# run-llama/semtools

Hardware: AMD Instinct MI355X
Metric: chunk-vectors scanned/sec (whole job) (higher is better)
Workload: dtype f32; 1 GPU; c2: 1 query x 1M chunks (D=256, f32) per GPU, brute-force cosine + top-k; rows_per_gpu=1000000, dim=256, top_k=10, corpus_copies_rotated=2

## Files before the change

### include/semtools_hip.h

```cpp
#ifndef SEMTOOLS_HIP_H
#define SEMTOOLS_HIP_H

#include <stdint.h>

#ifdef __cplusplus
extern "C" {
#endif

#define SMT_OK 0
#define SMT_E_INVALID (-1)
#define SMT_E_HIP (-2)
#define SMT_E_NOMEM (-3)
#define SMT_E_TRUNCATED (-4)
#define SMT_E_IO (-5)
#define SMT_E_UNSUPPORTED (-6)

#define SMT_DIM 256u

#define SMT_MODE_DOCUMENTS 0
#define SMT_MODE_WORKSPACE 1

typedef struct smt_ctx smt_ctx;
typedef struct smt_model smt_model;
typedef struct smt_corpus smt_corpus;
// ... 350 lines not shown

int smt_debug_scan_pairs(smt_ctx *ctx, uint64_t *paired, uint64_t *alone, uint64_t *absorbed);

int smt_debug_scan_groups(smt_ctx *ctx, uint64_t *by_size );

int smt_debug_scan_groups_wide(smt_ctx *ctx, uint64_t *by_size );

int smt_debug_scan_groups_deep(smt_ctx *ctx, uint64_t *by_size );

int smt_debug_select_groups(smt_ctx *ctx, uint64_t *by_size );

int smt_debug_ov_ready(smt_ctx *ctx, uint64_t *records);

int smt_debug_host_timing(smt_ctx *ctx, uint64_t *ns , uint64_t *calls);

#define SMT_DEBUG_FAIL_STAGE 1
#define SMT_DEBUG_FAIL_AGREE 2
#define SMT_DEBUG_FAIL_BUILD 3
int smt_debug_group_fail_next(smt_group *group, int where, int code);

int smt_debug_batched_scores(smt_corpus *corpus, const float *queries, uint32_t nq, uint64_t first_row, uint32_t n_rows,
                             float *out);

int smt_debug_nominations(smt_corpus *corpus, const float *queries, uint32_t nq, uint32_t top_k, const smt_range *ranges, uint32_t n_ranges,
                          const float *tau, int buffered, float *out_dist, uint32_t *out_hits, uint32_t *out_counts, uint32_t *out_route);

int smt_debug_merge_sources(smt_ctx *ctx, const uint64_t *const *lists_dev, uint32_t n_lists, uint32_t nq, uint32_t k_in, uint32_t k_out,
                            uint64_t *out_packed_dev);
int smt_debug_merge_packed_strided(smt_ctx *ctx, const uint64_t *packed_dev, uint64_t list_stride_words, uint32_t n_lists, uint32_t nq,
                                   uint32_t k_in, uint32_t k_out, uint64_t *out_packed_dev);
// ... 25 lines not shown
```

### rust/src/search/hip_ffi.rs

```rust
#![allow(non_camel_case_types, dead_code)]
use std::os::raw::{c_char, c_int, c_void};

macro_rules! opaque { ($($name:ident),*) => { $( #[repr(C)] pub struct $name { _private: [u8; 0] } )* } }
opaque!(SmtCtx, SmtModel, SmtCorpus, SmtIvfpq, SmtGroup, SmtShardedCorpus, SmtShardedIvfpq, SmtShardedModel, SmtWordpiece, SmtUnigram, SmtLower);

#[repr(C)]
#[derive(Clone, Copy, Debug, PartialEq, Eq)]
pub struct SmtRange {
    pub begin: u64,
    pub end: u64,
}

#[repr(C)]
#[derive(Clone, Copy, Debug, Default)]
pub struct SmtIvfpqParams {
    pub nlist: u32,
    pub m: u32,
    pub nbits: u32,
    pub train_iters: u32,
    pub train_sample: u64,
    pub reserved: u32,
    pub local_pca: u32,
}

// ... 872 lines not shown
    pub fn smt_debug_range_sets(corpus: *const SmtCorpus, kept: *mut u64, hits: *mut u64, builds: *mut u64) -> c_int;
    pub fn smt_debug_image_tile(
        corpus: *mut SmtCorpus,
        tile: u64,
        out_tile_host: *mut c_void,
        out_zero_mask: *mut u32,
    ) -> c_int;
    pub fn smt_debug_deliveries(ctx: *mut SmtCtx, count: *mut u64) -> c_int;
    pub fn smt_debug_scan_pairs(ctx: *mut SmtCtx, paired: *mut u64, alone: *mut u64, absorbed: *mut u64) -> c_int;
    pub fn smt_debug_scan_groups(ctx: *mut SmtCtx, by_size: *mut u64) -> c_int;
    pub fn smt_debug_scan_groups_wide(ctx: *mut SmtCtx, by_size: *mut u64) -> c_int;
    pub fn smt_debug_scan_groups_deep(ctx: *mut SmtCtx, by_size: *mut u64) -> c_int;
    pub fn smt_debug_select_groups(ctx: *mut SmtCtx, by_size: *mut u64) -> c_int;
    pub fn smt_debug_ov_ready(ctx: *mut SmtCtx, records: *mut u64) -> c_int;
    pub fn smt_debug_host_timing(ctx: *mut SmtCtx, ns: *mut u64, calls: *mut u64) -> c_int;
    pub fn smt_debug_group_fail_next(group: *mut SmtGroup, where_: c_int, code: c_int) -> c_int;
    pub fn smt_debug_batched_scores(
        corpus: *mut SmtCorpus,
        queries: *const f32,
        nq: u32,
        first_row: u64,
        n_rows: u32,
        out: *mut f32,
    ) -> c_int;
    pub fn smt_debug_nominations(
        corpus: *mut SmtCorpus,
        queries: *const f32,
        nq: u32,
        top_k: u32,
        ranges: *const SmtRange,
// ... 86 lines not shown
```

### semtools_amd/_lib.py

```python
import ctypes as C
import os
import subprocess

import numpy as np

_HERE = os.path.dirname(os.path.abspath(__file__))
LIB_PATH = os.path.join(_HERE, "lib", "libsemtools_hip.so")

SMT_OK, SMT_E_INVALID, SMT_E_HIP, SMT_E_NOMEM, SMT_E_TRUNCATED, SMT_E_IO, SMT_E_UNSUPPORTED = 0, -1, -2, -3, -4, -5, -6
MODE_DOCUMENTS, MODE_WORKSPACE = 0, 1
DIM = 256

EXPORTS = [
    "smt_ctx_create", "smt_ctx_create_on_stream", "smt_ctx_aux_stream", "smt_ctx_destroy", "smt_ctx_synchronize", "smt_last_error", "smt_version",
    "smt_device_count", "smt_prof_enable", "smt_prof_reset", "smt_prof_read",
    "smt_model_create", "smt_model_create_from_file", "smt_model_create_from_device", "smt_model_destroy", "smt_embed", "smt_embed_device",
    "smt_corpus_create", "smt_corpus_from_device", "smt_corpus_destroy", "smt_corpus_append_host",
    "smt_corpus_write_rows", "smt_corpus_read_rows", "smt_corpus_truncate", "smt_corpus_rows", "smt_corpus_dim",
    "smt_corpus_prepack", "smt_corpus_image_bytes",
    "smt_corpus_save", "smt_corpus_load", "smt_corpus_append_to_file", "smt_search", "smt_search_topk_device", "smt_merge_topk",
    "smt_merge_topk_device", "smt_merge_topk_packed_device", "smt_ivfpq_build", "smt_ivfpq_destroy", "smt_ivfpq_search", "smt_ivfpq_search_device", "smt_ivfpq_search_ranges", "smt_ivfpq_search_ranges_device", "smt_ivfpq_search_wide", "smt_ivfpq_search_wide_device", "smt_ivfpq_info", "smt_ivfpq_list_sizes", "smt_ivfpq_save", "smt_ivfpq_load", "smt_ivfpq_append", "smt_ivfpq_compact", "smt_sharded_ivfpq_compact",
    "smt_set_tuning", "smt_fnv1a_hash", "smt_line_embedding_id", "smt_doc_meta_id",
    "smt_ctx_uncertain_count", "smt_debug_batched_scores",
    "smt_init", "smt_shutdown", "smt_default_group", "smt_group_create", "smt_group_create_logical", "smt_group_unique_id", "smt_group_create_rank",
# ... 2 lines not shown
    "smt_sharded_corpus_destroy", "smt_sharded_corpus_rows", "smt_sharded_corpus_rank_rows", "smt_sharded_corpus_shard",
    "smt_sharded_corpus_append_host", "smt_sharded_search", "smt_sharded_search_topk_device",
    "smt_sharded_ivfpq_build", "smt_sharded_ivfpq_destroy", "smt_sharded_ivfpq_shard", "smt_sharded_ivfpq_search", "smt_sharded_ivfpq_search_ranges", "smt_sharded_ivfpq_search_wide",
    "smt_group_from_ctx", "smt_sharded_corpus_create", "smt_sharded_corpus_load_layout", "smt_sharded_corpus_layout",
    "smt_sharded_corpus_append_to_file", "smt_sharded_corpus_read_rows", "smt_sharded_corpus_write_rows",
    "smt_sharded_model_create", "smt_sharded_model_create_from_file", "smt_sharded_model_destroy", "smt_sharded_embed",
    "smt_sharded_ivfpq_save", "smt_sharded_ivfpq_load", "smt_sharded_ivfpq_append", "smt_sharded_ivfpq_info",
    "smt_group_set_transport", "smt_group_transport", "smt_debug_range_sets", "smt_sharded_corpus_append_to_file_ex",
    "smt_debug_group_fail_next", "smt_search_topk_device_ex", "smt_sharded_search_topk_device_ex", "smt_debug_deliveries",
    "smt_corpus_compact", "smt_ctx_compact_stats", "smt_sharded_corpus_compact",
    "smt_model_create_typed", "smt_model_create_from_file_typed", "smt_model_create_from_device_typed", "smt_model_info",
    "smt_sharded_model_create_typed", "smt_sharded_model_create_from_file_typed", "smt_sharded_model_info",
    "smt_model_create_indexed", "smt_model_create_from_file_indexed", "smt_model_create_from_device_indexed", "smt_model_token_info",
    "smt_sharded_model_create_indexed", "smt_sharded_model_create_from_file_indexed", "smt_sharded_model_token_info",
    "smt_debug_scan_pairs", "smt_debug_image_tile", "smt_debug_scan_groups", "smt_debug_scan_groups_wide", "smt_debug_scan_groups_deep","smt_debug_nominations",
    "smt_debug_select_groups", "smt_debug_ov_ready", "smt_debug_host_timing",
    "smt_debug_merge_sources", "smt_debug_merge_packed_strided", "smt_debug_combine_status", "smt_debug_select_lists",
    "smt_debug_scan_lists", "smt_debug_scan_ring",
    "smt_wordpiece_create", "smt_wordpiece_create_utf8", "smt_wordpiece_info", "smt_wordpiece_destroy", "smt_wordpiece_scan_device", "smt_wordpiece_emit_device", "smt_wordpiece_tokenize",
    "smt_unigram_create", "smt_unigram_create_utf8", "smt_unigram_info", "smt_unigram_destroy", "smt_unigram_scan_device", "smt_unigram_emit_device", "smt_unigram_tokenize",
    "smt_unigram_set_long_pieces", "smt_unigram_long_stats", "smt_unigram_set_space_rules", "smt_unigram_set_long_rules",
    "smt_lower_tables_check", "smt_lower_create", "smt_lower_destroy", "smt_lower_device", "smt_lower_lines",
]
WP_NORMALIZER, WP_CLEAN_TEXT, WP_LOWERCASE = 1, 2, 4
WP_CP_ORDINARY, WP_CP_SPACE, WP_CP_ALONE, WP_CP_DROPPED, WP_CP_FLAG = 0, 1, 2, 3, 4
UG_MAX_WORD = 64
UG_MAX_LONG = 2048
UG_PREPEND = {"always": 0, "first": 1, "never": 2}
TABLE_F32, TABLE_F16, TABLE_I8 = 0, 1, 2
TABLE_DTYPES = {np.dtype(np.float32): TABLE_F32, np.dtype(np.float16): TABLE_F16, np.dtype(np.int8): TABLE_I8}
TABLE_NP = {v: k for k, v in TABLE_DTYPES.items()}
# ... 240 lines not shown
    L.smt_group_synchronize.argtypes = [vp]
    L.smt_group_barrier.argtypes = [vp]
    try:
        L.smt_debug_range_sets.argtypes = [vp, P(C.c_uint64), P(C.c_uint64), P(C.c_uint64)]
        L.smt_debug_group_fail_next.argtypes = [vp, i32, i32]
        L.smt_debug_deliveries.argtypes = [vp, P(C.c_uint64)]
        L.smt_debug_scan_pairs.argtypes = [vp, P(C.c_uint64), P(C.c_uint64), P(C.c_uint64)]
        L.smt_debug_image_tile.argtypes = [vp, u64, vp, P(C.c_uint32)]
        L.smt_debug_scan_groups.argtypes = [vp, P(C.c_uint64)]
        L.smt_debug_nominations.argtypes = [vp, vp, u32, u32, vp, u32, vp, i32, vp, vp, vp, P(C.c_uint32)]
        L.smt_debug_scan_groups_wide.argtypes = [vp, P(C.c_uint64)]
        L.smt_debug_scan_groups_deep.argtypes = [vp, P(C.c_uint64)]
        L.smt_debug_select_groups.argtypes = [vp, P(C.c_uint64)]
        L.smt_debug_ov_ready.argtypes = [vp, P(C.c_uint64)]
        L.smt_debug_host_timing.argtypes = [vp, P(C.c_uint64), P(C.c_uint64)]
        L.smt_debug_merge_sources.argtypes = [vp, P(vp), u32, u32, u32, u32, vp]
        L.smt_debug_merge_packed_strided.argtypes = [vp, vp, u64, u32, u32, u32, u32, vp]
        L.smt_debug_combine_status.argtypes = [vp, P(vp), vp, u64, u32, u32, vp]
        L.smt_debug_select_lists.argtypes = [vp, vp, u32, vp, u64, u32, u32, u32, i32, C.c_float, u64, f64, vp, u64, vp, vp, vp, vp, vp]
        L.smt_debug_scan_lists.argtypes = [vp, vp, u32, u32, vp, u32, vp, u64, P(C.c_uint32), P(C.c_uint32), P(C.c_uint32)]
        L.smt_debug_scan_ring.argtypes = [vp, u32, u64, vp]
    except AttributeError:
        pass
    L.smt_sharded_corpus_append_to_file_ex.argtypes = [vp, C.c_char_p, u64, u64, i32]
    L.smt_group_set_transport.argtypes = [vp, i32]
    L.smt_group_transport.argtypes = [vp]
    L.smt_sharded_corpus_from_host.argtypes = [vp, vp, u64, u32, P(vp)]
    L.smt_sharded_corpus_from_device.argtypes = [vp, P(vp), P(u64), u32, P(vp)]
    L.smt_sharded_corpus_load.argtypes = [vp, C.c_char_p, P(vp)]
    L.smt_sharded_corpus_save.argtypes = [vp, C.c_char_p]
# ... 108 lines not shown
```

### semtools_amd/core.py

```python
import collections
import ctypes as C
import math

import numpy as np

from . import _lib as L


CompactStats = collections.namedtuple("CompactStats", "calls rows_moved")


def _f32c(a):
    return np.ascontiguousarray(a, dtype=np.float32)


def _table(a):
    if not isinstance(a, np.ndarray):
        return _f32c(a)
    L.table_dtype_code(a.dtype)
    return np.ascontiguousarray(a)


def _open(obj):
    return getattr(obj, "_h", None) is not None and bool(obj._h)
# ... 64 lines not shown

    def select_groups(self):
        v = (C.c_uint64 * 17)()
        L.check(L.lib().smt_debug_select_groups(self._h, v))
        return tuple(int(x) for x in v)

    def ov_ready_records(self):
        n = C.c_uint64(0)
        L.check(L.lib().smt_debug_ov_ready(self._h, C.byref(n)))
        return int(n.value)

    def host_timing(self):
        v, n = (C.c_uint64 * 8)(), C.c_uint64(0)
        L.check(L.lib().smt_debug_host_timing(self._h, v, C.byref(n)))
        return tuple(int(x) for x in v), int(n.value)

    def compact_stats(self, reset=False):
        n, m = C.c_uint64(0), C.c_uint64(0)
        L.check(L.lib().smt_ctx_compact_stats(self._h, C.byref(n), C.byref(m), int(bool(reset))))
        return CompactStats(int(n.value), int(m.value))

    def aux_stream(self):
        st = C.c_void_p()
        L.check(L.lib().smt_ctx_aux_stream(self._h, C.byref(st)))
        return int(st.value or 0)

    def set_tuning(self, key, value):
        L.check(L.lib().smt_set_tuning(self._h, key.encode(), int(value)))

    def prof_enable(self, on=True):
# ... 992 lines not shown
```

### semtools_amd/csrc/api.cpp

```cpp
#include <algorithm>
#include <cerrno>
#include <cmath>
#include <limits>
#include <string>

#include <unistd.h>

#include "common.h"

namespace smt {

static thread_local char g_err[512] = "";

void set_error(const char *fmt, ...)
{
    va_list ap;
    va_start(ap, fmt);
    vsnprintf(g_err, sizeof(g_err), fmt, ap);
    va_end(ap);
}

int ensure_scratch(smt_ctx *ctx, size_t bytes)
{
    if (bytes <= ctx->scratch_bytes) return SMT_OK;
// ... 47 lines not shown
{
    if (!ctx->aux_stream || !ctx->ov_stream[0]) return SMT_OK;
    for (int b = 0; b < 2; ++b) {
        SMT_HIP_CHECK(hipEventRecord(ctx->ov_sel[b], ctx->ov_stream[b]));
        SMT_HIP_CHECK(hipStreamWaitEvent(ctx->aux_stream, ctx->ov_sel[b], 0));
    }
    return SMT_OK;
}

int drain_async(smt_ctx *ctx)
{
    if (!ctx->async_pending) return SMT_OK;
    ctx->async_pending = false;
    for (hipStream_t st : ctx->ov_stream)
        if (st) SMT_HIP_CHECK(hipStreamSynchronize(st));
    if (ctx->pair_live) {
        ctx->pair_live = false;
        unsigned long long gave_up = 0;
        SMT_HIP_CHECK(hipMemcpy(&gave_up, ctx->d_gate + 1, sizeof(gave_up), hipMemcpyDeviceToHost));
        if (gave_up) {
            (void)hipMemset(ctx->d_gate + 1, 0, sizeof(gave_up));
            set_error("scan_pair: a scan block gave up waiting for its launch's grouping decision");
            return SMT_E_HIP;
        }
    }
    if (!ctx->aux_stream || !ctx->d_flags) return SMT_OK;
    SMT_HIP_CHECK(hipStreamSynchronize(ctx->stream));
    SMT_HIP_CHECK(hipStreamSynchronize(ctx->aux_stream));
    unsigned long long timed_out = 0;
    SMT_HIP_CHECK(hipMemcpy(&timed_out, ctx->d_flags + 3, sizeof(timed_out), hipMemcpyDeviceToHost));
// ... 280 lines not shown
    if (ctx->aux_stream) { (void)hipStreamSynchronize(ctx->aux_stream); (void)hipStreamDestroy(ctx->aux_stream); }
    for (int b = 0; b < 2; ++b) {
        if (ctx->ov_stream[b]) { (void)hipStreamSynchronize(ctx->ov_stream[b]); (void)hipStreamDestroy(ctx->ov_stream[b]); }
        if (ctx->ov_ready[b]) (void)hipEventDestroy(ctx->ov_ready[b]);
        if (ctx->ov_sel[b]) (void)hipEventDestroy(ctx->ov_sel[b]);
    }
    if (ctx->ov_done) (void)hipEventDestroy(ctx->ov_done);
    if (ctx->d_gate) (void)hipFree(ctx->d_gate);
    if (ctx->d_pair_recs) (void)hipFree(ctx->d_pair_recs);
    if (ctx->d_wide_recs) (void)hipFree(ctx->d_wide_recs);
    if (ctx->d_deep_recs) (void)hipFree(ctx->d_deep_recs);
    if (ctx->h_pair_ring) (void)hipHostFree(ctx->h_pair_ring);
    if (ctx->d_deep_sel_recs) (void)hipFree(ctx->d_deep_sel_recs);
    if (ctx->d_sel_groups) (void)hipFree(ctx->d_sel_groups);
    if (ctx->h_sel_ring) (void)hipHostFree(ctx->h_sel_ring);
    if (ctx->d_flags) (void)hipFree(ctx->d_flags);
    if (ctx->d_status) (void)hipFree(ctx->d_status);
    if (ctx->d_steal) (void)hipFree(ctx->d_steal);
    for (auto &kv : ctx->prof)
        for (hipEvent_t ev : kv.second.ev) (void)hipEventDestroy(ev);
    if (ctx->d_scratch) (void)hipFree(ctx->d_scratch);
    if (ctx->d_largek) (void)hipFree(ctx->d_largek);
    if (ctx->d_embed_runs) (void)hipFree(ctx->d_embed_runs);
    if (ctx->h_pinned) (void)hipHostFree(ctx->h_pinned);
    if (ctx->h_pinned_in) (void)hipHostFree(ctx->h_pinned_in);
    if (ctx->h_ivf_ranges) (void)hipHostFree(ctx->h_ivf_ranges);
    if (ctx->ivf_ranges_up) (void)hipEventDestroy(ctx->ivf_ranges_up);
    if (ctx->d_stage) (void)hipFree(ctx->d_stage);
    if (ctx->own_stream) (void)hipStreamDestroy(ctx->stream);
    delete ctx;
// ... 22 lines not shown
    return SMT_OK;
} catch (...) { return smt::api_catch(); }

int smt_debug_scan_pairs(smt_ctx *ctx, uint64_t *paired, uint64_t *alone, uint64_t *absorbed)
try {
    int rc = check_ctx(ctx);
    if (rc) return rc;
    SMT_REQUIRE(paired && alone && absorbed, "null argument");
    if ((rc = bind_device(ctx))) return rc;
    SMT_HIP_CHECK(hipStreamSynchronize(ctx->stream));
    if ((rc = sync_side_streams(ctx))) return rc;
    unsigned long long v[3] = {0, 0, 0};
    if (ctx->d_gate) SMT_HIP_CHECK(hipMemcpy(v, ctx->d_gate + 2, sizeof(v), hipMemcpyDeviceToHost));
    *paired = v[0];
    *alone = v[1] + ctx->pair_alone_host;
    *absorbed = v[2];
    return SMT_OK;
} catch (...) { return smt::api_catch(); }

int smt_debug_scan_groups(smt_ctx *ctx, uint64_t *by_size)
try {
    int rc = check_ctx(ctx);
    if (rc) return rc;
    SMT_REQUIRE(by_size != nullptr, "null argument");
    if ((rc = bind_device(ctx))) return rc;
    SMT_HIP_CHECK(hipStreamSynchronize(ctx->stream));
    if ((rc = sync_side_streams(ctx))) return rc;
    unsigned long long v[6] = {0, 0, 0, 0, 0, 0};
    if (ctx->d_gate) SMT_HIP_CHECK(hipMemcpy(v, ctx->d_gate + 2, sizeof(v), hipMemcpyDeviceToHost));
    by_size[0] = v[1] + ctx->pair_alone_host;
    by_size[1] = v[3];
// ... 30 lines not shown
    for (int n = 0; n < 16; ++n) by_size[n] = v[n];
    return SMT_OK;
} catch (...) { return smt::api_catch(); }

int smt_debug_select_groups(smt_ctx *ctx, uint64_t *by_size)
try {
    int rc = check_ctx(ctx);
    if (rc) return rc;
    SMT_REQUIRE(by_size != nullptr, "null argument");
    if ((rc = bind_device(ctx))) return rc;
    SMT_HIP_CHECK(hipStreamSynchronize(ctx->stream));
    if ((rc = sync_side_streams(ctx))) return rc;
    unsigned long long v[17] = {};
    if (ctx->d_sel_groups) SMT_HIP_CHECK(hipMemcpy(v, ctx->d_sel_groups, sizeof(v), hipMemcpyDeviceToHost));
    for (int n = 0; n < 17; ++n) by_size[n] = v[n];
    return SMT_OK;
} catch (...) { return smt::api_catch(); }

int smt_debug_ov_ready(smt_ctx *ctx, uint64_t *records)
try {
    int rc = check_ctx(ctx);
    if (rc) return rc;
    SMT_REQUIRE(records != nullptr, "null argument");
    *records = ctx->ov_ready_records;
    return SMT_OK;
} catch (...) { return smt::api_catch(); }

int smt_debug_host_timing(smt_ctx *ctx, uint64_t *ns, uint64_t *calls)
try {
    int rc = check_ctx(ctx);
// ... 132 lines not shown
        if (rc2) return rc2;
        SMT_REQUIRE(value >= 0 && value <= 15, "scan_deep: 0..15 later calls a queued scan may take along");
        ctx->tune.scan_pair = (int)value;
    } else if (k == "scan_pair_ring") {
        SMT_REQUIRE(value >= 64 && value <= 4096 && (value & (value - 1)) == 0, "scan_pair_ring: a power of two, 64..4096 slots");
        int rc2 = drain_async(ctx);
        if (rc2) return rc2;
        ctx->tune.scan_pair_ring = (int)value;
    } else if (k == "scan_pair_wait_us") {
        SMT_REQUIRE(value >= 0 && value <= 5000, "scan_pair_wait_us: 0..5000 us (tests only)");
        ctx->tune.scan_pair_wait_us = (int)value;
    } else if (k == "select_group") {
        int rc2 = drain_async(ctx);
        if (rc2) return rc2;
        ctx->tune.select_group = value ? 1 : 0;
    } else if (k == "ov_skip_ready") {
        ctx->tune.ov_skip_ready = value ? 1 : 0;
    } else if (k == "host_timing") {
        ctx->tune.host_timing = value ? 1 : 0;
        for (uint64_t &ns : ctx->host_ns) ns = 0;
        ctx->host_ns_calls = 0;
    } else if (k == "scan_gate_pct") {
        SMT_REQUIRE(value >= -1 && value <= 100, "scan_gate_pct: 0..100 per cent of the previous scan's blocks (0 = no gate), or -1 for the default");
        ctx->tune.scan_gate_pct = (int)value;
    }
    else if (k == "scan_debug_ptr") ctx->tune.scan_debug_ptr = value;
    else if (k == "select_debug_ptr") ctx->tune.select_debug_ptr = value;
    else if (k == "prof_select") ctx->tune.prof_select = (int)value;
    else if (k == "direct_delivery") ctx->tune.direct_delivery = (int)value;
    else if (k == "compact_bounce_rows") ctx->tune.compact_bounce_rows = std::max<int64_t>(64, std::min<int64_t>((int64_t)1 << 20, value));
// ... 436 lines not shown
```

### semtools_amd/csrc/common.h

```cpp
#pragma once

#include <hip/hip_runtime.h>

#include <cstdarg>
#include <cstdint>
#include <cstdio>
#include <cstring>
#include <map>
#include <string>
#include <vector>

#include "../../include/semtools_hip.h"

namespace smt {

void set_error(const char *fmt, ...);

#define SMT_HIP_CHECK(expr)                                                              \
    do {                                                                                 \
        hipError_t _e = (expr);                                                          \
        if (_e != hipSuccess) {                                                          \
            smt::set_error("%s failed: %s (%s:%d)", #expr, hipGetErrorString(_e),        \
                           __FILE__, __LINE__);                                          \
            return SMT_E_HIP;                                                            \
        }                                                                                \
    } while (0)

// ... 23 lines not shown
    int scan_unroll = 4;
    int scan_nontemporal = 1;
    int scan_prefetch = 1;
    int scan_steal = 0;
    int scan_steal_pct = 6;
    int gemm_blocks = 0;
    int prof_every = 1;
    int merge_on_aux = 0;
    int async_select = 0;
    int scan_overlap = 1;
    int scan_gate_pct = -1;
    int scan_pair = 15;
    int scan_pair_ring = 4096;
    int scan_pair_wait_us = 0;
    int select_group = 1;
    int ov_skip_ready = 1;
    int host_timing = 0;
    int gemm_image = 1;
    int64_t image_scan_min_rows = 1500000;
    int64_t image_use_min_rows = 400000;
    int corpus_image = 1;
    int embed_batched = 3;
    int gemm_split_last = 2;
    int gemm_boot_fine = 1;
    int gemm_bootstrap = 1;
    int gemm_buffered = 1;
    int gemm_qsplit = 1;
    int gemm_dma_nt = 1;
    int64_t fallback_batch_min_rows = 100000;
    int guard_band = 8;
// ... 50 lines not shown
    bool ov_lists_live = false;
    uint64_t gate_total = 0;
    uint64_t gate_prev_blocks = 0;
    uint64_t gate_prev_rows = 0;
    void *h_pair_ring = nullptr;
    void *d_pair_recs = nullptr;
    void *d_wide_recs = nullptr;
    void *d_deep_recs = nullptr;
    void *h_sel_ring = nullptr;
    void *d_deep_sel_recs = nullptr;
    unsigned long long *d_sel_groups = nullptr;
    uint64_t ov_ready_records = 0;
    uint64_t host_ns[8] = {};
    uint64_t host_ns_calls = 0;
    uint64_t pair_alone_host = 0;
    bool pair_live = false;
    unsigned int *d_steal = nullptr;
    uint64_t steal_seq = 0;
    unsigned long long deliver_seq = 0;
    uint64_t deliveries = 0;
    uint64_t compact_calls = 0;
    uint64_t compact_rows_moved = 0;
    bool prof_on = false;
    uint32_t attr_done = 0;
    std::map<std::string, smt::ProfEntry> prof;
    smt::Tuning tune;
};

namespace smt {
struct RangeSet {
// ... 318 lines not shown
```

### semtools_amd/csrc/scan_deep.hip

```cpp
#include "scan_group.h"

namespace smt {


__device__ __forceinline__ unsigned int deep_decide(const ScanParams &p, const DeepParams &pp, DeepRecord *rec, int lane)
{
    enum : int { SLOT_PENDING = 0, SLOT_PASS = 1, SLOT_FAIL = 2 };
    const unsigned long long t0 = wall_clock64();
    const unsigned long long want = p.step + 2ull * (unsigned long long)(lane + 1);
    const PairSlot *s = pp.ring + (want & pp.ring_mask);
    const unsigned long long expect = (unsigned long long)p.kp | pp.family | (unsigned long long)gridDim.x << 32;
    const SelSlot *ss = pp.sel_ring ? pp.sel_ring + (want & pp.ring_mask) : nullptr;
    int status = (unsigned int)lane < pp.max_take ? SLOT_PENDING : SLOT_FAIL;
    unsigned long long query = 0, lists = 0;
    SelSlot sel = {0, 0, 0, 0};
    unsigned int taken = 0;
    for (;;) {
        if (status == SLOT_PENDING) {
            const unsigned long long s1 = __hip_atomic_load(&s->step, __ATOMIC_ACQUIRE, __HIP_MEMORY_SCOPE_SYSTEM);
            if (s1 == want) {
                const unsigned long long corpus = sys_load(&s->corpus), n_virtual = sys_load(&s->n_virtual), kp_blocks = sys_load(&s->kp_blocks);
                const unsigned long long absorbable = sys_load(&s->absorbable);
                query = sys_load(&s->query);
                lists = sys_load(&s->lists);
                if (ss) {
                    sel.out_rows = sys_load(&ss->out_rows);
                    sel.out_dist = sys_load(&ss->out_dist);
                    sel.out_status = sys_load(&ss->out_status);
                    sel.row_base = sys_load(&ss->row_base);
                }
                __builtin_amdgcn_fence(__ATOMIC_ACQUIRE, "");
// ... 11 lines not shown
        __builtin_amdgcn_s_sleep(32);
    }
    if ((unsigned int)lane < taken) {
        flag_store(&rec->query[lane], query);
        flag_store(&rec->lists[lane], lists);
        if (ss) {
            SelSlot *m = &pp.sel_recs[p.step % DEEP_RECS].member[lane];
            flag_store(&m->out_rows, sel.out_rows);
            flag_store(&m->out_dist, sel.out_dist);
            flag_store(&m->out_status, sel.out_status);
            flag_store(&m->row_base, sel.row_base);
        }
        flag_store(&pp.recs[want % DEEP_RECS].state, (want << PAIR_SHIFT) | PAIR_ABSORBED);
    }
    if (lane == 0) flag_store(&rec->taken, (unsigned long long)taken);
    return taken;
}

template <bool NT>
__global__ void __launch_bounds__(512) __attribute__((amdgpu_waves_per_eu(8, 8))) scan_deep_kernel(ScanParams p, DeepParams pp)
{
    constexpr int U = 4;
    constexpr int NQ = DEEP_MAX;
    extern __shared__ unsigned char smem_raw[];
    key_t64 *s_list = reinterpret_cast<key_t64 *>(smem_raw);

    const int lane = threadIdx.x & 63;
    const int wave = __builtin_amdgcn_readfirstlane(threadIdx.x >> 6);
    const int waves_per_block = blockDim.x >> 6;
    f32x4 *s_rec = reinterpret_cast<f32x4 *>(s_list + NQ * SHARED_LIST_KEYS);
// ... 231 lines not shown
```

### semtools_amd/csrc/scan_group.h

```cpp
#pragma once
#include "scan_params.h"
#include "shared_list.h"

namespace smt {

constexpr int PAIR_RING = 4096;
constexpr int PAIR_RECS = 64;
constexpr int GROUP_MAX = 4;
constexpr int WIDE_MAX = 8;
constexpr int WIDE_RECS = 64;
constexpr int DEEP_MAX = 16;
constexpr int DEEP_RECS = 64;
constexpr unsigned long long WIDE_FAMILY = 1ull << 16;
constexpr unsigned long long DEEP_FAMILY = 1ull << 17;
struct PairSlot {
    unsigned long long step;
    unsigned long long corpus, n_virtual, query, lists;
    unsigned long long kp_blocks;
    unsigned long long absorbable;
    unsigned long long pad;
};
template <int MAX>
struct GroupRecord {
    unsigned long long state;
// ... 36 lines not shown
    unsigned int max_take;
    unsigned long long wait_ticks;
    unsigned long long ring_mask;
};
struct DeepParams {
    const PairSlot *ring;
    const SelSlot *sel_ring;
    DeepSelRecord *sel_recs;
    unsigned long long family;
    DeepRecord *recs;
    unsigned long long *ctl;
    unsigned int absorbable;
    unsigned int max_take;
    unsigned long long wait_ticks;
    unsigned long long ring_mask;
};
constexpr int DEEP_CTL_BY_SIZE = 11;

static inline size_t pair_smem_bytes(int threads)
{
    return (size_t)GROUP_MAX * (threads / 64) * 64 * sizeof(key_t64) + 256 + (size_t)GROUP_MAX * 1024 + 9 * 8 + 16;
}
static inline size_t wide_smem_bytes(int threads)
{
    return (size_t)WIDE_MAX * 32 * sizeof(key_t64) + (size_t)WIDE_MAX * 16 + 64 + (size_t)WIDE_MAX * 1024 + 18 * 8 + 16;
}
static inline size_t deep_smem_bytes(int threads)
{
    return (size_t)DEEP_MAX * 32 * sizeof(key_t64) + (size_t)DEEP_MAX * 16 + 64 + (size_t)DEEP_MAX * 1024 + 34 * 8 + 16;
}
// ... 164 lines not shown
```

### semtools_amd/csrc/scan_launch.hip

```cpp
#include "scan_group.h"

namespace smt {

static inline uint32_t candidates_per_list(const smt_ctx *ctx, uint32_t k_out)
{
    return std::min<uint32_t>(64, k_out + (uint32_t)ctx->tune.guard_band);
}

struct HostTimer {
    smt_ctx *ctx;
    bool on;
    timespec t;
    explicit HostTimer(smt_ctx *c) : ctx(c), on(c->tune.host_timing != 0)
    {
        if (on) clock_gettime(CLOCK_MONOTONIC, &t);
    }
    void lap(int kind)
    {
        if (!on) return;
        timespec n;
        clock_gettime(CLOCK_MONOTONIC, &n);
        ctx->host_ns[kind] += (uint64_t)((n.tv_sec - t.tv_sec) * 1000000000ll + (n.tv_nsec - t.tv_nsec));
        t = n;
    }
// ... 6 lines not shown
    uint64_t n_chunks;
    bool async, overlap;
    bool pair;
    uint64_t step = 0;
    key_t64 *lists = nullptr;
    uint64_t *table = nullptr;
    hipStream_t st = nullptr;
    unsigned long long gate_open = 0, gate_ticks = 0;
    bool may_pair = false;
    bool wide = false;
    bool deep = false;
    unsigned int absorbable = 0;
    bool sel_group = false;
    SelSlot sel = {0, 0, 0, 0};
    uint32_t sel_k_out = 0;
};

static ScanPlan plan_scan(const smt_ctx *ctx, const ScanArgs &a)
{
    ScanPlan pl;
    pl.filtered = a.n_ranges > 0;
    pl.nt = ctx->tune.scan_nontemporal != 0;
    pl.kp = candidates_per_list(ctx, a.k_out);
    pl.blocks = ctx->tune.scan_blocks > 0 ? ctx->tune.scan_blocks : ctx->num_cus;
    if (pl.blocks > SEL_MAX_LISTS) pl.blocks = SEL_MAX_LISTS;
    pl.threads = ctx->tune.scan_threads;
    pl.U = pl.filtered ? FILTER_CHUNK : ctx->tune.scan_unroll;
    pl.n_chunks = pl.filtered ? a.n_chunks : (a.n_virtual + (uint64_t)pl.U - 1) / (uint64_t)pl.U;
    const uint64_t waves_per_block = (uint64_t)(pl.threads / 64);
    if ((uint64_t)pl.blocks * waves_per_block > pl.n_chunks) {
// ... 109 lines not shown
int ensure_pair(smt_ctx *ctx)
{
    if (ctx->h_pair_ring) return SMT_OK;
    SMT_HIP_CHECK(hipMalloc(&ctx->d_pair_recs, PAIR_RECS * sizeof(PairRecord)));
    SMT_HIP_CHECK(hipMemset(ctx->d_pair_recs, 0, PAIR_RECS * sizeof(PairRecord)));
    SMT_HIP_CHECK(hipMalloc(&ctx->d_wide_recs, WIDE_RECS * sizeof(WideRecord)));
    SMT_HIP_CHECK(hipMemset(ctx->d_wide_recs, 0, WIDE_RECS * sizeof(WideRecord)));
    SMT_HIP_CHECK(hipMalloc(&ctx->d_deep_recs, DEEP_RECS * sizeof(DeepRecord)));
    SMT_HIP_CHECK(hipMemset(ctx->d_deep_recs, 0, DEEP_RECS * sizeof(DeepRecord)));
    SMT_HIP_CHECK(hipMalloc(&ctx->d_deep_sel_recs, DEEP_RECS * sizeof(DeepSelRecord)));
    SMT_HIP_CHECK(hipMemset(ctx->d_deep_sel_recs, 0, DEEP_RECS * sizeof(DeepSelRecord)));
    SMT_HIP_CHECK(hipMalloc(reinterpret_cast<void **>(&ctx->d_sel_groups), (GROUP_SEL_MAX + 1) * sizeof(unsigned long long)));
    SMT_HIP_CHECK(hipMemset(ctx->d_sel_groups, 0, (GROUP_SEL_MAX + 1) * sizeof(unsigned long long)));
    SMT_HIP_CHECK(hipHostMalloc(&ctx->h_sel_ring, PAIR_RING * sizeof(SelSlot), hipHostMallocDefault));
    memset(ctx->h_sel_ring, 0, PAIR_RING * sizeof(SelSlot));
    SMT_HIP_CHECK(hipHostMalloc(&ctx->h_pair_ring, PAIR_RING * sizeof(PairSlot), hipHostMallocDefault));
    memset(ctx->h_pair_ring, 0, PAIR_RING * sizeof(PairSlot));
    return SMT_OK;
}

static unsigned long long group_family(const ScanPlan &pl)
{
    if (pl.wide) return WIDE_FAMILY;
    if (!pl.deep) return 0ull;
    return DEEP_FAMILY | (pl.sel_group ? DEEP_SELGROUP | (unsigned long long)pl.sel_k_out << DEEP_KOUT_SHIFT : 0ull);
}

static unsigned long long pair_ring_mask(const smt_ctx *ctx)
{
    return (unsigned long long)std::min(ctx->tune.scan_pair_ring, PAIR_RING) - 1;
// ... 19 lines not shown
{
    PP pp{};
    pp.absorbable = pl.absorbable;
    pp.ring_mask = pair_ring_mask(ctx);
    pp.ring = reinterpret_cast<const PairSlot *>(ctx->h_pair_ring);
    pp.recs = reinterpret_cast<decltype(pp.recs)>(recs);
    pp.ctl = ctx->d_gate + 1;
    pp.wait_ticks = (unsigned long long)ctx->tune.scan_pair_wait_us * 100ull;
    pp.max_take = (unsigned int)std::min(std::max(ctx->tune.scan_pair, 1), max_take);
    return pp;
}

static int launch_scan_pair(smt_ctx *ctx, const ScanParams &p, const ScanPlan &pl)
{
    publish_slot(ctx, p, pl);
    if (pl.deep) {
        DeepParams dp = group_params<DeepParams>(ctx, pl, ctx->d_deep_recs, DEEP_MAX - 1);
        dp.family = group_family(pl);
        if (pl.sel_group) {
            dp.sel_ring = reinterpret_cast<const SelSlot *>(ctx->h_sel_ring);
            dp.sel_recs = reinterpret_cast<DeepSelRecord *>(ctx->d_deep_sel_recs);
        }
        launch_scan_deep_kernel(pl.nt, pl.blocks, pl.threads, pl.st, p, dp);
    } else if (pl.wide) {
        launch_scan_wide_kernel(pl.nt, pl.blocks, pl.threads, pl.st, p, group_params<WideParams>(ctx, pl, ctx->d_wide_recs, WIDE_MAX - 1));
    } else {
        launch_scan_pair_kernel(pl.nt, pl.blocks, pl.threads, pl.st, p, group_params<PairParams>(ctx, pl, ctx->d_pair_recs, GROUP_MAX - 1));
    }
    SMT_HIP_CHECK(hipGetLastError());
    ctx->pair_live = true;
    return SMT_OK;
}

static int launch_scan_pass(smt_ctx *ctx, const ScanPlan &pl, const ScanParams &p, int slots)
{
    if (slots == 1 && pl.pair) {
        if (pl.may_pair) return launch_scan_pair(ctx, p, pl);
        ++ctx->pair_alone_host;
    }
    launch_scan_topk_kernel(slots, pl.U, pl.nt, pl.filtered, pl.blocks, pl.threads, pl.st, p);
    SMT_HIP_CHECK(hipGetLastError());
    return SMT_OK;
}

static SelectArgs select_args(const ScanArgs &a, const ScanPlan &pl)
{
    SelectArgs s;
    s.corpus = a.corpus;
    s.queries = a.queries;
    s.nq = a.nq;
    s.lists = pl.lists;
    s.n_lists = (uint32_t)pl.blocks;
    s.kp = pl.kp;
    s.list_stride = (uint64_t)pl.blocks * pl.kp;
    s.k_out = a.k_out;
    s.ws_threshold = a.ws_threshold;
// ... 44 lines not shown
    int rc = scan_begin(ctx, a, pl);
    if (rc != SMT_OK) return rc;
    HostTimer whole(ctx);
    if (pl.overlap && (rc = overlap_prologue(ctx, pl))) return rc;
    const SelectArgs sa = select_args(a, pl);
    if (pl.deep && pl.may_pair && ctx->tune.select_group) {
        pl.sel_group = group_select_serves(sa);
        if (pl.sel_group) {
            pl.sel = SelSlot{(unsigned long long)(uintptr_t)sa.out_rows, (unsigned long long)(uintptr_t)sa.out_dist,
                             (unsigned long long)(uintptr_t)sa.out_status, (unsigned long long)sa.row_base};
            pl.sel_k_out = sa.k_out;
        } else {
            pl.absorbable = 0;
        }
    }
    HostTimer ht(ctx);

    prof_begin_on(ctx, "scan", pl.st);
    if ((rc = scan_passes(ctx, a, pl, nullptr))) return rc;
    prof_end_on(ctx, "scan", pl.st);

    if (pl.overlap) {
        ctx->gate_total += (uint64_t)pl.blocks;
        ctx->gate_prev_blocks = (uint64_t)pl.blocks;
        ctx->gate_prev_rows = a.n_virtual;
        ctx->async_pending = true;
        ctx->async_overlap = true;
    } else if (pl.async) {
        ctx->async_overlap = false;
    }
    ht.lap(2);
    if (pl.sel_group) {
        GroupSelect gs;
        gs.rec = reinterpret_cast<const unsigned long long *>(reinterpret_cast<const DeepRecord *>(ctx->d_deep_recs) + pl.step % DEEP_RECS);
        gs.sel = reinterpret_cast<const unsigned long long *>(reinterpret_cast<const DeepSelRecord *>(ctx->d_deep_sel_recs) + pl.step % DEEP_RECS);
        gs.absorbed = (pl.step << PAIR_SHIFT) | PAIR_ABSORBED;
        gs.paired = (pl.step << PAIR_SHIFT) | PAIR_PAIRED;
        gs.hist = ctx->d_sel_groups;
        rc = launch_group_select(ctx, sa, gs);
    } else {
        rc = launch_select(ctx, sa);
    }
    ht.lap(3);
    if (rc == SMT_OK && pl.overlap && ctx->aux_stream) {
        SMT_HIP_CHECK(hipEventRecord(ctx->ov_sel[pl.step & 1], pl.st));
        SMT_HIP_CHECK(hipStreamWaitEvent(ctx->aux_stream, ctx->ov_sel[pl.step & 1], 0));
    }
// ... 44 lines not shown
```

Baseline: 53.81 billion rows/s.

## Let host skip kernel launches for calls a running deep-scan leader will absorb

Adds a host-side take protocol. When an overlapped deep-group scan is live, later compatible calls are recorded as members and skip both the scan kernel launch and the select launch. This only happens while a pinned 'closing' word written by the leader kernel shows the leader has not yet closed its intake. The leader kernel now publishes its closing step and how many calls it took. The host checks those counts later and raises an error if the leader took fewer calls than expected. This is meant to remove per-call launch overhead, at the cost of fence and spin logic on host-device shared memory and a new failure mode.

```diff
diff --git a/include/semtools_hip.h b/include/semtools_hip.h
--- a/include/semtools_hip.h
+++ b/include/semtools_hip.h
@@ -388,6 +388,8 @@
 
 int smt_debug_host_timing(smt_ctx *ctx, uint64_t *ns , uint64_t *calls);
 
+int smt_debug_host_taken(smt_ctx *ctx, uint64_t *taken, uint64_t *guard_waits);
+
 #define SMT_DEBUG_FAIL_STAGE 1
 #define SMT_DEBUG_FAIL_AGREE 2
 #define SMT_DEBUG_FAIL_BUILD 3
diff --git a/rust/src/search/hip_ffi.rs b/rust/src/search/hip_ffi.rs
--- a/rust/src/search/hip_ffi.rs
+++ b/rust/src/search/hip_ffi.rs
@@ -910,6 +910,7 @@
     pub fn smt_debug_select_groups(ctx: *mut SmtCtx, by_size: *mut u64) -> c_int;
     pub fn smt_debug_ov_ready(ctx: *mut SmtCtx, records: *mut u64) -> c_int;
     pub fn smt_debug_host_timing(ctx: *mut SmtCtx, ns: *mut u64, calls: *mut u64) -> c_int;
+    pub fn smt_debug_host_taken(ctx: *mut SmtCtx, taken: *mut u64, guard_waits: *mut u64) -> c_int;
     pub fn smt_debug_group_fail_next(group: *mut SmtGroup, where_: c_int, code: c_int) -> c_int;
     pub fn smt_debug_batched_scores(
         corpus: *mut SmtCorpus,
diff --git a/semtools_amd/_lib.py b/semtools_amd/_lib.py
--- a/semtools_amd/_lib.py
+++ b/semtools_amd/_lib.py
@@ -40,7 +40,7 @@
     "smt_model_create_indexed", "smt_model_create_from_file_indexed", "smt_model_create_from_device_indexed", "smt_model_token_info",
     "smt_sharded_model_create_indexed", "smt_sharded_model_create_from_file_indexed", "smt_sharded_model_token_info",
     "smt_debug_scan_pairs", "smt_debug_image_tile", "smt_debug_scan_groups", "smt_debug_scan_groups_wide", "smt_debug_scan_groups_deep","smt_debug_nominations",
-    "smt_debug_select_groups", "smt_debug_ov_ready", "smt_debug_host_timing",
+    "smt_debug_select_groups", "smt_debug_ov_ready", "smt_debug_host_timing", "smt_debug_host_taken",
     "smt_debug_merge_sources", "smt_debug_merge_packed_strided", "smt_debug_combine_status", "smt_debug_select_lists",
     "smt_debug_scan_lists", "smt_debug_scan_ring",
     "smt_wordpiece_create", "smt_wordpiece_create_utf8", "smt_wordpiece_info", "smt_wordpiece_destroy", "smt_wordpiece_scan_device", "smt_wordpiece_emit_device", "smt_wordpiece_tokenize",
@@ -311,6 +311,7 @@
         L.smt_debug_select_groups.argtypes = [vp, P(C.c_uint64)]
         L.smt_debug_ov_ready.argtypes = [vp, P(C.c_uint64)]
         L.smt_debug_host_timing.argtypes = [vp, P(C.c_uint64), P(C.c_uint64)]
+        L.smt_debug_host_taken.argtypes = [vp, P(C.c_uint64), P(C.c_uint64)]
         L.smt_debug_merge_sources.argtypes = [vp, P(vp), u32, u32, u32, u32, vp]
         L.smt_debug_merge_packed_strided.argtypes = [vp, vp, u64, u32, u32, u32, u32, vp]
         L.smt_debug_combine_status.argtypes = [vp, P(vp), vp, u64, u32, u32, vp]
diff --git a/semtools_amd/core.py b/semtools_amd/core.py
--- a/semtools_amd/core.py
+++ b/semtools_amd/core.py
@@ -102,6 +102,11 @@
         v, n = (C.c_uint64 * 8)(), C.c_uint64(0)
         L.check(L.lib().smt_debug_host_timing(self._h, v, C.byref(n)))
         return tuple(int(x) for x in v), int(n.value)
+
+    def host_taken(self):
+        t, g = C.c_uint64(0), C.c_uint64(0)
+        L.check(L.lib().smt_debug_host_taken(self._h, C.byref(t), C.byref(g)))
+        return int(t.value), int(g.value)
 
     def compact_stats(self, reset=False):
         n, m = C.c_uint64(0), C.c_uint64(0)
diff --git a/semtools_amd/csrc/api.cpp b/semtools_amd/csrc/api.cpp
--- a/semtools_amd/csrc/api.cpp
+++ b/semtools_amd/csrc/api.cpp
@@ -85,6 +85,10 @@
     ctx->async_pending = false;
     for (hipStream_t st : ctx->ov_stream)
         if (st) SMT_HIP_CHECK(hipStreamSynchronize(st));
+    if (take_has_state(ctx->host_take) && take_drain(ctx->host_take) != TAKE_OK) {
+        set_error("host_take: a leader took fewer calls than the host had counted on");
+        return SMT_E_HIP;
+    }
     if (ctx->pair_live) {
         ctx->pair_live = false;
         unsigned long long gave_up = 0;
@@ -395,6 +399,7 @@
     if (ctx->d_deep_sel_recs) (void)hipFree(ctx->d_deep_sel_recs);
     if (ctx->d_sel_groups) (void)hipFree(ctx->d_sel_groups);
     if (ctx->h_sel_ring) (void)hipHostFree(ctx->h_sel_ring);
+    if (ctx->host_take.words) (void)hipHostFree(ctx->host_take.words);
     if (ctx->d_flags) (void)hipFree(ctx->d_flags);
     if (ctx->d_status) (void)hipFree(ctx->d_status);
     if (ctx->d_steal) (void)hipFree(ctx->d_steal);
@@ -447,7 +452,7 @@
     if (ctx->d_gate) SMT_HIP_CHECK(hipMemcpy(v, ctx->d_gate + 2, sizeof(v), hipMemcpyDeviceToHost));
     *paired = v[0];
     *alone = v[1] + ctx->pair_alone_host;
-    *absorbed = v[2];
+    *absorbed = v[2] + ctx->host_take.taken;
     return SMT_OK;
 } catch (...) { return smt::api_catch(); }
 
@@ -508,6 +513,17 @@
     unsigned long long v[17] = {};
     if (ctx->d_sel_groups) SMT_HIP_CHECK(hipMemcpy(v, ctx->d_sel_groups, sizeof(v), hipMemcpyDeviceToHost));
     for (int n = 0; n < 17; ++n) by_size[n] = v[n];
+    by_size[0] += ctx->host_take.taken;
+    return SMT_OK;
+} catch (...) { return smt::api_catch(); }
+
+int smt_debug_host_taken(smt_ctx *ctx, uint64_t *taken, uint64_t *guard_waits)
+try {
+    int rc = check_ctx(ctx);
+    if (rc) return rc;
+    SMT_REQUIRE(taken != nullptr && guard_waits != nullptr, "null argument");
+    *taken = ctx->host_take.taken;
+    *guard_waits = ctx->host_take.guard_waits;
     return SMT_OK;
 } catch (...) { return smt::api_catch(); }
 
@@ -670,6 +686,10 @@
         int rc2 = drain_async(ctx);
         if (rc2) return rc2;
         ctx->tune.select_group = value ? 1 : 0;
+    } else if (k == "host_take") {
+        int rc2 = drain_async(ctx);
+        if (rc2) return rc2;
+        ctx->tune.host_take = value ? 1 : 0;
     } else if (k == "ov_skip_ready") {
         ctx->tune.ov_skip_ready = value ? 1 : 0;
     } else if (k == "host_timing") {
diff --git a/semtools_amd/csrc/common.h b/semtools_amd/csrc/common.h
--- a/semtools_amd/csrc/common.h
+++ b/semtools_amd/csrc/common.h
@@ -11,6 +11,7 @@
 #include <vector>
 
 #include "../../include/semtools_hip.h"
+#include "host_take.h"
 
 namespace smt {
 
@@ -64,6 +65,7 @@
     int scan_pair_ring = 4096;
     int scan_pair_wait_us = 0;
     int select_group = 1;
+    int host_take = 1;
     int ov_skip_ready = 1;
     int host_timing = 0;
     int gemm_image = 1;
@@ -144,6 +146,7 @@
     uint64_t host_ns[8] = {};
     uint64_t host_ns_calls = 0;
     uint64_t pair_alone_host = 0;
+    smt::HostTake host_take;
     bool pair_live = false;
     unsigned int *d_steal = nullptr;
     uint64_t steal_seq = 0;
diff --git a/semtools_amd/csrc/host_take.h b/semtools_amd/csrc/host_take.h
--- /dev/null
+++ b/semtools_amd/csrc/host_take.h
@@ -0,0 +1,159 @@
+#pragma once
+#include <cstdint>
+#include <ctime>
+
+namespace smt {
+
+#ifndef SMT_HOST_TAKE_FENCE
+#define SMT_HOST_TAKE_FENCE() __atomic_thread_fence(__ATOMIC_SEQ_CST)
+#endif
+
+constexpr int TAKE_PENDING_MAX = 128;
+constexpr int TAKE_WORD_SHIFT = 8;
+enum : int { TAKE_OK = 0, TAKE_TIMEOUT = 1, TAKE_LOST = 2 };
+
+struct TakeWord {
+    unsigned long long closed;
+    unsigned long long taken;
+};
+struct TakeKey {
+    unsigned long long corpus, n_virtual, kp_blocks;
+};
+struct TakeAnchor {
+    bool live = false;
+    unsigned long long step = 0;
+    unsigned int members = 0, max_take = 0;
+    TakeKey key = {0, 0, 0};
+};
+struct TakePending {
+    unsigned long long step;
+    unsigned int members;
+};
+struct HostTake {
+    TakeWord *words = nullptr;
+    unsigned long long ring_mask = 0;
+    TakeAnchor cur[2];
+    TakePending pend[2][TAKE_PENDING_MAX];
+    unsigned int pend_head[2] = {0, 0}, pend_n[2] = {0, 0};
+    unsigned long long last_taken = 0;
+    unsigned long long taken = 0, guard_waits = 0, lost = 0;
+};
+
+inline bool take_has_state(const HostTake &t)
+{
+    return t.cur[0].live || t.cur[1].live || t.pend_n[0] || t.pend_n[1];
+}
+inline bool take_decided(const HostTake &t, unsigned long long step, unsigned int *taken)
+{
+    const unsigned long long w = __atomic_load_n(&t.words[step & t.ring_mask].taken, __ATOMIC_ACQUIRE);
+    if ((w >> TAKE_WORD_SHIFT) != step) return false;
+    *taken = (unsigned int)(w & ((1u << TAKE_WORD_SHIFT) - 1));
+    return true;
+}
+inline int take_check(HostTake &t, unsigned int members, unsigned int taken)
+{
+    if (members <= taken) return TAKE_OK;
+    ++t.lost;
+    return TAKE_LOST;
+}
+inline int take_reap(HostTake &t, int b)
+{
+    int rc = TAKE_OK;
+    unsigned int taken = 0;
+    while (t.pend_n[b] && take_decided(t, t.pend[b][t.pend_head[b]].step, &taken)) {
+        if (take_check(t, t.pend[b][t.pend_head[b]].members, taken)) rc = TAKE_LOST;
+        t.pend_head[b] = (t.pend_head[b] + 1) % TAKE_PENDING_MAX;
+        --t.pend_n[b];
+    }
+    return rc;
+}
+inline int take_wait(HostTake &t, unsigned long long step, unsigned int *taken, long long limit_ns)
+{
+    if (take_decided(t, step, taken)) return TAKE_OK;
+    ++t.guard_waits;
+    timespec t0, t1;
+    clock_gettime(CLOCK_MONOTONIC, &t0);
+    for (;;) {
+        for (int i = 0; i < 64; ++i) {
+            if (take_decided(t, step, taken)) return TAKE_OK;
+#if defined(__x86_64__) || defined(__i386__)
+            __builtin_ia32_pause();
+#endif
+        }
+        clock_gettime(CLOCK_MONOTONIC, &t1);
+        if ((t1.tv_sec - t0.tv_sec) * 1000000000ll + (t1.tv_nsec - t0.tv_nsec) > limit_ns) return TAKE_TIMEOUT;
+    }
+}
+inline void take_drop(HostTake &t, int b)
+{
+    TakeAnchor &a = t.cur[b];
+    if (!a.live) return;
+    a.live = false;
+    if (a.members == 0 || t.pend_n[b] == TAKE_PENDING_MAX) return;
+    t.pend[b][(t.pend_head[b] + t.pend_n[b]) % TAKE_PENDING_MAX] = TakePending{a.step, a.members};
+    ++t.pend_n[b];
+}
+inline int take_begin(HostTake &t, unsigned long long step, long long limit_ns)
+{
+    const int b = (int)(step & 1);
+    const unsigned long long ring = t.ring_mask + 1;
+    int rc = take_reap(t, b);
+    unsigned int taken = 0;
+    while (rc == TAKE_OK && t.pend_n[b] &&
+           (step - t.pend[b][t.pend_head[b]].step >= ring || t.pend_n[b] == TAKE_PENDING_MAX)) {
+        if ((rc = take_wait(t, t.pend[b][t.pend_head[b]].step, &taken, limit_ns))) return rc;
+        rc = take_reap(t, b);
+    }
+    TakeAnchor &a = t.cur[b];
+    if (rc == TAKE_OK && a.live && step - a.step >= ring) {
+        if ((rc = take_wait(t, a.step, &taken, limit_ns))) return rc;
+        rc = take_check(t, a.members, taken);
+        a.live = false;
+    }
+    return rc;
+}
+inline bool take_candidate(const HostTake &t, unsigned long long step, const TakeKey &key, bool absorbable)
+{
+    const TakeAnchor &a = t.cur[step & 1];
+    return a.live && absorbable && a.members < a.max_take && step == a.step + 2ull * (a.members + 1) && key.corpus == a.key.corpus &&
+           key.n_virtual == a.key.n_virtual && key.kp_blocks == a.key.kp_blocks;
+}
+inline void take_anchor(HostTake &t, unsigned long long step, const TakeKey &key, unsigned int max_take)
+{
+    TakeAnchor &a = t.cur[step & 1];
+    a.live = true;
+    a.step = step;
+    a.members = 0;
+    a.max_take = max_take;
+    a.key = key;
+}
+inline bool take_prove(HostTake &t, unsigned long long step)
+{
+    const int b = (int)(step & 1);
+    TakeAnchor &a = t.cur[b];
+    SMT_HOST_TAKE_FENCE();
+    if (__atomic_load_n(&t.words[a.step & t.ring_mask].closed, __ATOMIC_SEQ_CST) != a.step) {
+        ++a.members;
+        ++t.taken;
+        t.last_taken = step;
+        return true;
+    }
+    take_drop(t, b);
+    return false;
+}
+inline int take_drain(HostTake &t)
+{
+    int rc = TAKE_OK;
+    unsigned int taken = 0;
+    for (int b = 0; b < 2; ++b) {
+        take_drop(t, b);
+        for (; t.pend_n[b]; --t.pend_n[b], t.pend_head[b] = (t.pend_head[b] + 1) % TAKE_PENDING_MAX) {
+            const TakePending &p = t.pend[b][t.pend_head[b]];
+            if (!take_decided(t, p.step, &taken)) taken = 0;
+            if (take_check(t, p.members, taken)) rc = TAKE_LOST;
+        }
+    }
+    return rc;
+}
+
+}
diff --git a/semtools_amd/csrc/scan_deep.hip b/semtools_amd/csrc/scan_deep.hip
--- a/semtools_amd/csrc/scan_deep.hip
+++ b/semtools_amd/csrc/scan_deep.hip
@@ -15,6 +15,10 @@
     unsigned long long query = 0, lists = 0;
     SelSlot sel = {0, 0, 0, 0};
     unsigned int taken = 0;
+    if (pp.closing) {
+        if (lane == 0) __hip_atomic_store(pp.closing, p.step, __ATOMIC_SEQ_CST, __HIP_MEMORY_SCOPE_SYSTEM);
+        __builtin_amdgcn_fence(__ATOMIC_SEQ_CST, "");
+    }
     for (;;) {
         if (status == SLOT_PENDING) {
             const unsigned long long s1 = __hip_atomic_load(&s->step, __ATOMIC_ACQUIRE, __HIP_MEMORY_SCOPE_SYSTEM);
@@ -56,6 +60,8 @@
         flag_store(&pp.recs[want % DEEP_RECS].state, (want << PAIR_SHIFT) | PAIR_ABSORBED);
     }
     if (lane == 0) flag_store(&rec->taken, (unsigned long long)taken);
+    if (pp.closing && lane == 0)
+        __hip_atomic_store(pp.closing + 1, p.step << TAKE_WORD_SHIFT | (unsigned long long)taken, __ATOMIC_RELAXED, __HIP_MEMORY_SCOPE_SYSTEM);
     return taken;
 }
 
diff --git a/semtools_amd/csrc/scan_group.h b/semtools_amd/csrc/scan_group.h
--- a/semtools_amd/csrc/scan_group.h
+++ b/semtools_amd/csrc/scan_group.h
@@ -74,6 +74,7 @@
     unsigned int max_take;
     unsigned long long wait_ticks;
     unsigned long long ring_mask;
+    unsigned long long *closing;
 };
 constexpr int DEEP_CTL_BY_SIZE = 11;
 
diff --git a/semtools_amd/csrc/scan_launch.hip b/semtools_amd/csrc/scan_launch.hip
--- a/semtools_amd/csrc/scan_launch.hip
+++ b/semtools_amd/csrc/scan_launch.hip
@@ -44,6 +44,8 @@
     bool sel_group = false;
     SelSlot sel = {0, 0, 0, 0};
     uint32_t sel_k_out = 0;
+    enum : int { TAKE_NO = 0, TAKE_ANCHOR = 1, TAKE_CANDIDATE = 2 };
+    int take_role = TAKE_NO;
 };
 
 static ScanPlan plan_scan(const smt_ctx *ctx, const ScanArgs &a)
@@ -183,6 +185,9 @@
     SMT_HIP_CHECK(hipMemset(ctx->d_sel_groups, 0, (GROUP_SEL_MAX + 1) * sizeof(unsigned long long)));
     SMT_HIP_CHECK(hipHostMalloc(&ctx->h_sel_ring, PAIR_RING * sizeof(SelSlot), hipHostMallocDefault));
     memset(ctx->h_sel_ring, 0, PAIR_RING * sizeof(SelSlot));
+    if (!ctx->host_take.words)
+        SMT_HIP_CHECK(hipHostMalloc(reinterpret_cast<void **>(&ctx->host_take.words), PAIR_RING * sizeof(TakeWord), hipHostMallocDefault));
+    memset(ctx->host_take.words, 0, PAIR_RING * sizeof(TakeWord));
     SMT_HIP_CHECK(hipHostMalloc(&ctx->h_pair_ring, PAIR_RING * sizeof(PairSlot), hipHostMallocDefault));
     memset(ctx->h_pair_ring, 0, PAIR_RING * sizeof(PairSlot));
     return SMT_OK;
@@ -232,9 +237,12 @@
 static int launch_scan_pair(smt_ctx *ctx, const ScanParams &p, const ScanPlan &pl)
 {
     publish_slot(ctx, p, pl);
+    if (pl.take_role == ScanPlan::TAKE_CANDIDATE && take_prove(ctx->host_take, p.step)) return SMT_OK;
     if (pl.deep) {
         DeepParams dp = group_params<DeepParams>(ctx, pl, ctx->d_deep_recs, DEEP_MAX - 1);
         dp.family = group_family(pl);
+        if (pl.take_role == ScanPlan::TAKE_ANCHOR)
+            dp.closing = reinterpret_cast<unsigned long long *>(ctx->host_take.words + (p.step & pair_ring_mask(ctx)));
         if (pl.sel_group) {
             dp.sel_ring = reinterpret_cast<const SelSlot *>(ctx->h_sel_ring);
             dp.sel_recs = reinterpret_cast<DeepSelRecord *>(ctx->d_deep_sel_recs);
@@ -258,6 +266,33 @@
     }
     launch_scan_topk_kernel(slots, pl.U, pl.nt, pl.filtered, pl.blocks, pl.threads, pl.st, p);
     SMT_HIP_CHECK(hipGetLastError());
+    return SMT_OK;
+}
+
+static int host_take_role(smt_ctx *ctx, const ScanArgs &a, ScanPlan &pl)
+{
+    HostTake &t = ctx->host_take;
+    const bool active = pl.sel_group && ctx->tune.host_take && ctx->tune.scan_pair_wait_us == 0 && !(ctx->prof_on && ctx->tune.prof_select);
+    if (!active && !take_has_state(t)) return SMT_OK;
+    t.ring_mask = pair_ring_mask(ctx);
+    int rc = take_begin(t, pl.step, 100000000ll);
+    if (rc == TAKE_TIMEOUT && (rc = drain_async(ctx))) return rc;
+    if (rc == TAKE_LOST) {
+        set_error("host_take: a leader took fewer calls than the host had counted on");
+        return SMT_E_HIP;
+    }
+    const TakeKey key = {(unsigned long long)(uintptr_t)a.corpus, a.n_virtual,
+                         (unsigned long long)pl.kp | group_family(pl) | (unsigned long long)pl.blocks << 32};
+    if (active && take_candidate(t, pl.step, key, pl.absorbable != 0)) {
+        pl.take_role = ScanPlan::TAKE_CANDIDATE;
+        return SMT_OK;
+    }
+    take_drop(t, (int)(pl.step & 1));
+    if (active) {
+        pl.take_role = ScanPlan::TAKE_ANCHOR;
+        pl.absorbable = 0;
+        take_anchor(t, pl.step, key, (unsigned int)std::min(std::max(ctx->tune.scan_pair, 1), DEEP_MAX - 1));
+    }
     return SMT_OK;
 }
 
@@ -332,11 +367,16 @@
             pl.absorbable = 0;
         }
     }
+    if (pl.overlap && (rc = host_take_role(ctx, a, pl))) return rc;
     HostTimer ht(ctx);
 
     prof_begin_on(ctx, "scan", pl.st);
-    if ((rc = scan_passes(ctx, a, pl, nullptr))) return rc;
+    if ((rc = scan_passes(ctx, a, pl, nullptr))) {
+        if (pl.take_role == ScanPlan::TAKE_ANCHOR) ctx->host_take.cur[pl.step & 1].live = false;
+        return rc;
+    }
     prof_end_on(ctx, "scan", pl.st);
+    const bool taken = pl.take_role == ScanPlan::TAKE_CANDIDATE && ctx->host_take.last_taken == pl.step;
 
     if (pl.overlap) {
         ctx->gate_total += (uint64_t)pl.blocks;
@@ -348,7 +388,8 @@
         ctx->async_overlap = false;
     }
     ht.lap(2);
-    if (pl.sel_group) {
+    if (taken) {
+    } else if (pl.sel_group) {
         GroupSelect gs;
         gs.rec = reinterpret_cast<const unsigned long long *>(reinterpret_cast<const DeepRecord *>(ctx->d_deep_recs) + pl.step % DEEP_RECS);
         gs.sel = reinterpret_cast<const unsigned long long *>(reinterpret_cast<const DeepSelRecord *>(ctx->d_deep_sel_recs) + pl.step % DEEP_RECS);
```

Measured after the change: 53.54 billion rows/s. Within noise of the previous version (-0.5%).
